# dhansmair/flamingo-mini

Hardware: AMD Instinct MI355X
Metric: images/sec (fwd+bwd) flamingo-mini bs=32 (higher is better)
Workload: dtype bf16

## Files before the change

flamingo-mini_amd/csrc/ff_rowwise.hip:

```cpp
#include "ff_common.h"
#include "ff_internal.h"

namespace ff {

#ifdef FF_XA_TIMELINE
__device__ unsigned long long g_ln_timeline[4096 * 8];
#define FF_LTL(i) do { if (threadIdx.x == 0 && blockIdx.x < 4096) g_ln_timeline[blockIdx.x * 8 + (i)] = __builtin_amdgcn_s_memrealtime(); } while (0)
#else
#define FF_LTL(i) do { } while (0)
#endif

template <typename T, int VEC> FF_DEV void ld(const T* p, float (&o)[VEC]) {
    if constexpr (VEC == 1) o[0] = to_f32(p[0]);
    else Vec<T>::load(p, o);
}
template <typename T, int VEC> FF_DEV void st(T* p, const float (&o)[VEC]) {
    if constexpr (VEC == 1) p[0] = from_f32<T>(o[0]);
    else Vec<T>::store(p, o);
}

template <typename T, int VEC>
__global__ __launch_bounds__(256) void ln_fwd_kernel(const LnArgs a_in, const T* __restrict__ x, const T* __restrict__ add,
                                                     const T* __restrict__ gamma, const T* __restrict__ beta, T* __restrict__ y,
                                                     float* __restrict__ mean, float* __restrict__ rstd) {
    const LnArgs a = fetch_args(a_in);
    pin_args(x, add, gamma, beta, y, mean, rstd);
    const int lane = threadIdx.x & 63;
    const int row = blockIdx.x * 4 + (threadIdx.x >> 6);
    if (row >= a.rows) return;
    const T* xr = x + a.x_map.off(row);
    const T* ar = nullptr;
    if (add) ar = add + (long long)((row % a.add_rows_per_seg) / a.add_div) * a.cols;
    const int nchunk = a.cols / VEC;
    float mu, rs;
    if (nchunk <= 4 * 64 && VEC > 1) {
        float v[4][VEC];
#pragma unroll
        for (int u = 0; u < 4; u++) {
            const int c = lane + 64 * u;
            if (c < nchunk) {
                ld<T, VEC>(xr + c * VEC, v[u]);
                if (ar) {
                    float t[VEC];
                    ld<T, VEC>(ar + c * VEC, t);
#pragma unroll
                    for (int i = 0; i < VEC; i++) v[u][i] += t[i];
                }
            }
        }
        if (a.stats_given) {
            mu = mean[row];
            rs = rstd[row];
        } else {
            float s = 0.f;
#pragma unroll
            for (int u = 0; u < 4; u++)
                if (lane + 64 * u < nchunk)
#pragma unroll
                    for (int i = 0; i < VEC; i++) s += v[u][i];
            mu = wave_sum(s) / (float)a.cols;
            float q = 0.f;
#pragma unroll
            for (int u = 0; u < 4; u++)
                if (lane + 64 * u < nchunk)
#pragma unroll
                    for (int i = 0; i < VEC; i++) q += (v[u][i] - mu) * (v[u][i] - mu);
            rs = rsqrtf(wave_sum(q) / (float)a.cols + a.eps);
            if (lane == 0 && mean) {
                mean[row] = mu;
                rstd[row] = rs;
            }
        }
        if (!y) return;
        T* yr = y + a.y_map.off(row);
#pragma unroll
        for (int u = 0; u < 4; u++) {
            const int c = lane + 64 * u;
            if (c < nchunk) {
                float g[VEC], b[VEC], o[VEC];
                ld<T, VEC>(gamma + c * VEC, g);
                ld<T, VEC>(beta + c * VEC, b);
#pragma unroll
                for (int i = 0; i < VEC; i++) o[i] = (v[u][i] - mu) * rs * g[i] + b[i];
                st<T, VEC>(yr + c * VEC, o);
            }
        }
        return;
    }
    if (a.stats_given) {
        mu = mean[row];
        rs = rstd[row];
    } else {
        float s = 0.f;
        for (int c = lane; c < nchunk; c += 64) {
            float v[VEC];
            ld<T, VEC>(xr + c * VEC, v);
            if (ar) {
                float t[VEC];
                ld<T, VEC>(ar + c * VEC, t);
#pragma unroll
                for (int i = 0; i < VEC; i++) v[i] += t[i];
            }
#pragma unroll
            for (int i = 0; i < VEC; i++) s += v[i];
        }
        mu = wave_sum(s) / (float)a.cols;
        float q = 0.f;
        for (int c = lane; c < nchunk; c += 64) {
            float v[VEC];
            ld<T, VEC>(xr + c * VEC, v);
            if (ar) {
                float t[VEC];
                ld<T, VEC>(ar + c * VEC, t);
#pragma unroll
                for (int i = 0; i < VEC; i++) v[i] += t[i];
            }
#pragma unroll
            for (int i = 0; i < VEC; i++) q += (v[i] - mu) * (v[i] - mu);
        }
        rs = rsqrtf(wave_sum(q) / (float)a.cols + a.eps);
        if (lane == 0 && mean) {
            mean[row] = mu;
            rstd[row] = rs;
        }
    }
    if (!y) return;
    T* yr = y + a.y_map.off(row);
    for (int c = lane; c < nchunk; c += 64) {
        float v[VEC], g[VEC], b[VEC];
        ld<T, VEC>(xr + c * VEC, v);
        if (ar) {
            float t[VEC];
            ld<T, VEC>(ar + c * VEC, t);
#pragma unroll
            for (int i = 0; i < VEC; i++) v[i] += t[i];
        }
        ld<T, VEC>(gamma + c * VEC, g);
        ld<T, VEC>(beta + c * VEC, b);
#pragma unroll
        for (int i = 0; i < VEC; i++) v[i] = (v[i] - mu) * rs * g[i] + b[i];
        st<T, VEC>(yr + c * VEC, v);
    }
}

template <typename T, int VEC>
__global__ __launch_bounds__(256) void ln_bwd_dx_kernel(const LnArgs a_in, const T* __restrict__ dy, const T* __restrict__ x,
                                                        const T* __restrict__ add, const T* __restrict__ gamma,
                                                        const float* __restrict__ mean, const float* __restrict__ rstd, T* dx,
                                                        const T* dx_res) {
    const LnArgs a = fetch_args(a_in);
    pin_args(dy, x, add, gamma, mean, rstd, dx, dx_res);
    const int lane = threadIdx.x & 63;
    const int row = blockIdx.x * 4 + (threadIdx.x >> 6);
    if (row >= a.rows) return;
    const T* xr = x + a.x_map.off(row);
    const T* dyr = dy + a.y_map.off(row);
    const T* ar = nullptr;
    if (add) ar = add + (long long)((row % a.add_rows_per_seg) / a.add_div) * a.cols;
    const float mu = mean[row], rs = rstd[row];
    const int nchunk = a.cols / VEC;
    float s1 = 0.f, s2 = 0.f;
    for (int c = lane; c < nchunk; c += 64) {
        float v[VEC], d[VEC], g[VEC];
        ld<T, VEC>(xr + c * VEC, v);
        if (ar) {
            float t[VEC];
            ld<T, VEC>(ar + c * VEC, t);
#pragma unroll
            for (int i = 0; i < VEC; i++) v[i] += t[i];
        }
        ld<T, VEC>(dyr + c * VEC, d);
        ld<T, VEC>(gamma + c * VEC, g);
#pragma unroll
        for (int i = 0; i < VEC; i++) {
            const float dyh = d[i] * g[i];
            s1 += dyh;
            s2 += dyh * (v[i] - mu) * rs;
        }
    }
    const float m1 = wave_sum(s1) / (float)a.cols, m2 = wave_sum(s2) / (float)a.cols;
    const long long doff = a.dx_map.off(row);
    for (int c = lane; c < nchunk; c += 64) {
        float v[VEC], d[VEC], g[VEC], o[VEC];
        ld<T, VEC>(xr + c * VEC, v);
        if (ar) {
            float t[VEC];
            ld<T, VEC>(ar + c * VEC, t);
#pragma unroll
            for (int i = 0; i < VEC; i++) v[i] += t[i];
        }
        ld<T, VEC>(dyr + c * VEC, d);
        ld<T, VEC>(gamma + c * VEC, g);
#pragma unroll
        for (int i = 0; i < VEC; i++) o[i] = rs * (d[i] * g[i] - m1 - (v[i] - mu) * rs * m2);
        if (dx_res) {
            float q[VEC];
            ld<T, VEC>(dx_res + doff + c * VEC, q);
#pragma unroll
            for (int i = 0; i < VEC; i++) o[i] += q[i];
        }
        st<T, VEC>(dx + doff + c * VEC, o);
    }
}


template <typename T, int VEC, int NCH>
__global__ __launch_bounds__(256) void ln_bwd_fused_kernel(const LnArgs a_in, const T* __restrict__ dy, const T* __restrict__ x,
                                                           const T* __restrict__ add, const T* __restrict__ gamma,
                                                           const float* __restrict__ mean, const float* __restrict__ rstd, T* dx,
                                                           const T* dx_res, const T* __restrict__ dot_a, const T* __restrict__ dot_b,
                                                           float* __restrict__ partial, int rows_per_block) {
    FF_LTL(0);
    const LnArgs a = fetch_args(a_in);
    pin_args(dy, x, add, gamma, mean, rstd, dx, dx_res, dot_a, dot_b, partial, rows_per_block);
    extern __shared__ __attribute__((aligned(16))) float sacc[];
    FF_LTL(1);
    __shared__ float red[4];
    const int lane = threadIdx.x & 63, w = threadIdx.x >> 6;
    const int nchunk = a.cols / VEC;
    float accg[NCH][VEC], accb[NCH][VEC];
#pragma unroll
    for (int i = 0; i < NCH; i++)
#pragma unroll
        for (int e = 0; e < VEC; e++) accg[i][e] = accb[i][e] = 0.f;
    float da = 0.f, db = 0.f;
    const int row_end = min(a.rows, (int)(blockIdx.x + 1) * rows_per_block);
    auto load_dy = [&](int row, const T* dyr, int c, float (&d)[VEC]) {
        if (a.dy_splits > 0) {
            const float* pp = (const float*)dy + (long long)row * a.cols + c * VEC;
#pragma unroll
            for (int e = 0; e < VEC; e++) d[e] = 0.f;
            for (int sp = 0; sp < a.dy_splits; sp++) {
#pragma unroll
                for (int e = 0; e < VEC; e += 4) {
                    const f32x4 q = *(const f32x4*)(pp + (long long)sp * a.dy_slab + e);
                    d[e] += q[0]; d[e + 1] += q[1]; d[e + 2] += q[2]; d[e + 3] += q[3];
                }
            }
        } else ld<T, VEC>(dyr + c * VEC, d);
    };
    for (int row = blockIdx.x * rows_per_block + w; row < row_end; row += 4) {
        const T* xr = x + a.x_map.off(row);
        const T* dyr = a.dy_splits > 0 ? dy : dy + a.y_map.off(row);
        const T* ar = add ? add + (long long)((row % a.add_rows_per_seg) / a.add_div) * a.cols : nullptr;
        const float mu = mean[row], rs = rstd[row];
        float s1 = 0.f, s2 = 0.f;
        constexpr bool KEEP = NCH <= 4;
        constexpr bool HOIST = KEEP && VEC > 1;
        float xk[KEEP ? NCH : 1][VEC], dk[KEEP ? NCH : 1][VEC];
        uint4 rq[HOIST ? NCH : 1], ra[HOIST ? NCH : 1], rb[HOIST ? NCH : 1];
        const long long doff = a.dx_map.off(row);
#pragma unroll
        for (int i = 0; i < NCH; i++) {
            const int c = lane + 64 * i;
            if (c < nchunk) {
                float v[VEC], d[VEC], g[VEC];
                ld<T, VEC>(xr + c * VEC, v);
                if (ar) {
                    float t[VEC];
                    ld<T, VEC>(ar + c * VEC, t);
#pragma unroll
                    for (int e = 0; e < VEC; e++) v[e] += t[e];
                }
                load_dy(row, dyr, c, d);
                ld<T, VEC>(gamma + c * VEC, g);
                if constexpr (HOIST) {
                    if (dx_res) rq[i] = *(const uint4*)(dx_res + doff + c * VEC);
                    if (dot_a) ra[i] = *(const uint4*)(dot_a + doff + c * VEC);
                    if (dot_b) rb[i] = *(const uint4*)(dot_b + doff + c * VEC);
                }
#pragma unroll
                for (int e = 0; e < VEC; e++) {
                    const float dyh = d[e] * g[e], xh = (v[e] - mu) * rs;
                    s1 += dyh;
                    s2 += dyh * xh;
                    if (KEEP) { xk[i][e] = xh; dk[i][e] = d[e]; }
                }
            }
        }
        const float m1 = wave_sum(s1) / (float)a.cols, m2 = wave_sum(s2) / (float)a.cols;
        auto unpack = [](const uint4& r, float (&o)[VEC]) {
            if constexpr (VEC > 1) {
                typedef typename Vec<T>::raw raw_t;
                const raw_t x = __builtin_bit_cast(raw_t, r);
#pragma unroll
                for (int e = 0; e < VEC; e++) o[e] = to_f32(x[e]);
            }
        };
#pragma unroll
        for (int i = 0; i < NCH; i++) {
            const int c = lane + 64 * i;
            if (c < nchunk) {
                float xh[VEC], d[VEC], g[VEC], o[VEC];
                if (KEEP) {
#pragma unroll
                    for (int e = 0; e < VEC; e++) { xh[e] = xk[i][e]; d[e] = dk[i][e]; }
                } else {
                    float v[VEC];
                    ld<T, VEC>(xr + c * VEC, v);
                    if (ar) {
                        float t[VEC];
                        ld<T, VEC>(ar + c * VEC, t);
#pragma unroll
                        for (int e = 0; e < VEC; e++) v[e] += t[e];
                    }
                    load_dy(row, dyr, c, d);
#pragma unroll
                    for (int e = 0; e < VEC; e++) xh[e] = (v[e] - mu) * rs;
                }
                ld<T, VEC>(gamma + c * VEC, g);
#pragma unroll
                for (int e = 0; e < VEC; e++) {
                    o[e] = rs * (d[e] * g[e] - m1 - xh[e] * m2);
                    accg[i][e] += d[e] * xh[e];
                    accb[i][e] += d[e];
                }
                if (dx_res) {
                    float q[VEC];
                    if constexpr (HOIST) unpack(rq[i], q);
                    else ld<T, VEC>(dx_res + doff + c * VEC, q);
                    if (dot_a) {
                        float u[VEC];
                        if constexpr (HOIST) unpack(ra[i], u);
                        else ld<T, VEC>(dot_a + doff + c * VEC, u);
#pragma unroll
                        for (int e = 0; e < VEC; e++) da += q[e] * u[e];
                    }
#pragma unroll
                    for (int e = 0; e < VEC; e++) o[e] += q[e];
                }
                if (dx) {
                    float r[VEC];
#pragma unroll
                    for (int e = 0; e < VEC; e++) r[e] = to_f32(from_f32<T>(o[e]));
                    if (dot_b) {
                        float u[VEC];
                        if constexpr (HOIST) unpack(rb[i], u);
                        else ld<T, VEC>(dot_b + doff + c * VEC, u);
#pragma unroll
                        for (int e = 0; e < VEC; e++) db += r[e] * u[e];
                    }
                    st<T, VEC>(dx + doff + c * VEC, o);
                }
            }
        }
    }
    FF_LTL(2);
    {
        float* mine = sacc + (size_t)w * 2 * a.cols;
#pragma unroll
        for (int i = 0; i < NCH; i++) {
            const int c = lane + 64 * i;
            if (c < nchunk) {
#pragma unroll
                for (int e = 0; e < VEC; e += 4) {
                    *(f32x4*)(mine + c * VEC + e) = f32x4{accg[i][e], accg[i][e + 1], accg[i][e + 2], accg[i][e + 3]};
                    *(f32x4*)(mine + a.cols + c * VEC + e) = f32x4{accb[i][e], accb[i][e + 1], accb[i][e + 2], accb[i][e + 3]};
                }
            }
        }
    }
    __syncthreads();
    FF_LTL(3);
    const long long P = 2LL * a.cols + 2;
    float* out = partial + (long long)blockIdx.x * P;
    for (int i = threadIdx.x * 4; i < 2 * a.cols; i += 256 * 4) {
        const f32x4 s0 = *(const f32x4*)(sacc + i), s1 = *(const f32x4*)(sacc + 2 * a.cols + i);
        const f32x4 s2 = *(const f32x4*)(sacc + 4 * a.cols + i), s3 = *(const f32x4*)(sacc + 6 * a.cols + i);
        float* o = out + i;
        o[0] = (s0[0] + s1[0]) + (s2[0] + s3[0]); o[1] = (s0[1] + s1[1]) + (s2[1] + s3[1]);
        o[2] = (s0[2] + s1[2]) + (s2[2] + s3[2]); o[3] = (s0[3] + s1[3]) + (s2[3] + s3[3]);
    }
    da = block_sum<4>(da, red);
    db = block_sum<4>(db, red);
    if (threadIdx.x == 0) { out[2 * a.cols] = da; out[2 * a.cols + 1] = db; }
    FF_LTL(4);
}

template <typename T>
FF_DEV void ln_final_body(int nblk, int cols, const float* __restrict__ partial, T* dgamma, T* dbeta, const T* alpha_a, T* out_a, const T* alpha_b,
                          T* out_b) {
    __shared__ float red[16][17];
    const int P = 2 * cols + 2;
    const int tx = threadIdx.x & 15, ty = threadIdx.x >> 4;
    const int idx = blockIdx.x * 16 + tx;
    float v[8] = {0.f, 0.f, 0.f, 0.f, 0.f, 0.f, 0.f, 0.f};
    if (idx < P) {
        int b = ty;
        for (; b + 7 * 16 < nblk; b += 8 * 16) {
#pragma unroll
            for (int u = 0; u < 8; u++) v[u] += partial[(long long)(b + 16 * u) * P + idx];
        }
        for (; b < nblk; b += 16) v[0] += partial[(long long)b * P + idx];
    }
    red[ty][tx] = ((v[0] + v[1]) + (v[2] + v[3])) + ((v[4] + v[5]) + (v[6] + v[7]));
    __syncthreads();
    if (ty == 0 && idx < P) {
        float s = 0.f;
#pragma unroll
        for (int u = 0; u < 16; u++) s += red[u][tx];
        const float v = s;
        if (idx < cols) { if (dgamma) dgamma[idx] = from_f32<T>(v); }
        else if (idx < 2 * cols) { if (dbeta) dbeta[idx - cols] = from_f32<T>(v); }
        else if (idx == 2 * cols) {
            if (out_a) { const float t = tanhf(to_f32(alpha_a[0])); out_a[0] = from_f32<T>(v * (1.f - t * t)); }
        } else if (out_b) { const float t = tanhf(to_f32(alpha_b[0])); out_b[0] = from_f32<T>(v * (1.f - t * t)); }
    }
}
template <typename T>
// ... 9 lines not shown
__global__ __launch_bounds__(256) void ln_bwd_final_multi_kernel(const LnFinishTable t) {
    const LnPending& e = t.s[blockIdx.y];
    if ((int)blockIdx.x * 16 >= 2 * e.cols + 2) return;
    ln_final_body<T>(e.nblk, e.cols, e.partial, (T*)e.dgamma, (T*)e.dbeta, (const T*)e.alpha_a, (T*)e.out_a, (const T*)e.alpha_b, (T*)e.out_b);
}

struct ColReduceArgs {
    int rows, cols;
    RowMap x_map, y_map;
    int rows_per_batch, rows_per_group, n_batch;
    int add_rows_per_seg, add_div;
    int rows_per_split, nsplit, ngroups;
};

template <typename T, int VEC, int MODE>
__global__ __launch_bounds__(256) void col_reduce_kernel(const ColReduceArgs a_in, const T* __restrict__ x, const T* __restrict__ dy,
                                                         const T* __restrict__ add, const float* __restrict__ mean,
                                                         const float* __restrict__ rstd, float* __restrict__ partial) {
    const ColReduceArgs a = fetch_args(a_in);
    pin_args(x, dy, add, mean, rstd, partial);
    constexpr int NS = MODE == 1 ? 2 : 1;
    __shared__ float red[4][NS][64 * VEC];
    const int tx = threadIdx.x & 63, ty = threadIdx.x >> 6;
    const int col = (blockIdx.x * 64 + tx) * VEC;
    const int g = blockIdx.y, split = blockIdx.z;
    float acc[NS][VEC];
#pragma unroll
    for (int s = 0; s < NS; s++)
#pragma unroll
        for (int i = 0; i < VEC; i++) acc[s][i] = 0.f;
    if (col < a.cols) {
        const int n_g = a.n_batch * a.rows_per_group;
        const int i_end = min(n_g, (split + 1) * a.rows_per_split);
        for (int i = split * a.rows_per_split + ty; i < i_end; i += 4) {
            const int bi = i / a.rows_per_group, j = i - bi * a.rows_per_group;
            const int row = bi * a.rows_per_batch + g * a.rows_per_group + j;
            if (row >= a.rows) continue;
            float v[VEC];
            ld<T, VEC>(x + a.x_map.off(row) + col, v);
            if (MODE == 0) {
#pragma unroll
                for (int e = 0; e < VEC; e++) acc[0][e] += v[e];
            } else {
                if (add) {
                    float t[VEC];
                    ld<T, VEC>(add + (long long)((row % a.add_rows_per_seg) / a.add_div) * a.cols + col, t);
#pragma unroll
                    for (int e = 0; e < VEC; e++) v[e] += t[e];
                }
                float d[VEC];
                ld<T, VEC>(dy + a.y_map.off(row) + col, d);
                const float mu = mean[row], rs = rstd[row];
#pragma unroll
                for (int e = 0; e < VEC; e++) {
                    acc[0][e] += d[e] * (v[e] - mu) * rs;
                    acc[1][e] += d[e];
                }
            }
        }
    }
#pragma unroll
    for (int s = 0; s < NS; s++)
#pragma unroll
        for (int e = 0; e < VEC; e++) red[ty][s][tx * VEC + e] = acc[s][e];
    __syncthreads();
    if (ty == 0 && col < a.cols) {
#pragma unroll
        for (int s = 0; s < NS; s++)
#pragma unroll
            for (int e = 0; e < VEC; e++) {
                const float v = red[0][s][tx * VEC + e] + red[1][s][tx * VEC + e] + red[2][s][tx * VEC + e] + red[3][s][tx * VEC + e];
                partial[(((long long)split * a.ngroups + g) * NS + s) * a.cols + col + e] = v;
            }
    }
}

template <typename T>
__global__ __launch_bounds__(256) void col_reduce_final_kernel(int nsplit, int ngroups, int nslots, int cols,
                                                               const float* __restrict__ partial, T* out0, T* out1) {
    pin_args(nsplit, ngroups, nslots, cols, partial, out0, out1);
    const long long total = (long long)ngroups * nslots * cols;
    for (long long idx = (long long)blockIdx.x * 256 + threadIdx.x; idx < total; idx += (long long)gridDim.x * 256) {
        float v0 = 0.f, v1 = 0.f, v2 = 0.f, v3 = 0.f;
        int s = 0;
        for (; s + 4 <= nsplit; s += 4) {
            v0 += partial[(long long)s * total + idx];
            v1 += partial[(long long)(s + 1) * total + idx];
            v2 += partial[(long long)(s + 2) * total + idx];
            v3 += partial[(long long)(s + 3) * total + idx];
        }
        for (; s < nsplit; s++) v0 += partial[(long long)s * total + idx];
        const float v = (v0 + v1) + (v2 + v3);
        const int c = (int)(idx % cols);
        const long long gs = idx / cols;
        const int slot = (int)(gs % nslots), g = (int)(gs / nslots);
        T* out = slot == 0 ? out0 : out1;
        out[(long long)g * cols + c] = from_f32<T>(v);
    }
}

template <typename T, int VEC>
__global__ __launch_bounds__(256) void dot_partial_kernel(long long n, const T* __restrict__ a, const T* __restrict__ b,
                                                          float* __restrict__ partial) {
    pin_args(n, a, b, partial);
    __shared__ float red[4];
// ... 36 lines not shown
              size_t ws_bytes, hipStream_t st_);

static bool vec_ok(int dtype, int cols, std::initializer_list<RowMap> maps, std::initializer_list<const void*> ptrs) {
    const int n = dtype == FF_DTYPE_BF16 ? 8 : 4;
    if (cols % n) return false;
    for (const RowMap& m : maps)
        if (m.ld % n || (m.rows_per_seg > 0 && m.seg_stride % n)) return false;
    for (const void* p : ptrs)
        if (p && (uintptr_t)p % 16) return false;
    return true;
}

#define FF_DISPATCH_T_VEC(dtype, vec, ...)                 \
    do {                                                    \
        if ((dtype) == FF_DTYPE_BF16) {                     \
            typedef bf16 T;                                 \
            if (vec) { constexpr int VEC = 8; __VA_ARGS__; }       \
            else { constexpr int VEC = 1; __VA_ARGS__; }           \
        } else {                                            \
            typedef float T;                                \
            if (vec) { constexpr int VEC = 4; __VA_ARGS__; }       \
            else { constexpr int VEC = 1; __VA_ARGS__; }           \
        }                                                   \
    } while (0)

int layernorm_fwd(const LnArgs& a, const void* x, const void* add, const void* gamma, const void* beta, void* y, float* mean,
                  float* rstd, hipStream_t st_) {
    FF_CHECK(a.rows > 0 && a.cols > 0 && x, FF_ERR_SHAPE, "layernorm_fwd: bad shape rows=%d cols=%d", a.rows, a.cols);
    FF_CHECK(!a.stats_given || (mean && rstd), FF_ERR_SHAPE, "layernorm_fwd: stats_given without statistics");
    FF_CHECK(!y || (gamma && beta), FF_ERR_SHAPE, "layernorm_fwd: gamma/beta missing");
    FF_CHECK(!add || (a.add_rows_per_seg > 0 && a.add_div > 0), FF_ERR_SHAPE, "layernorm_fwd: addend needs add_rows_per_seg/add_div");
    const bool v = vec_ok(a.dtype, a.cols, {a.x_map, a.y_map}, {x, add, gamma, beta, y});
    const int grid = cdiv(a.rows, 4);
    FF_DISPATCH_T_VEC(a.dtype, v, ln_fwd_kernel<T, VEC><<<dim3(grid), dim3(256), 0, st_>>>(a, (const T*)x, (const T*)add, (const T*)gamma, (const T*)beta, (T*)y, mean, rstd));
    return check_launch("ln_fwd");
}

static void split_plan(int n_rows_in_group, int col_blocks, int ngroups, int& rows_per_split, int& nsplit) {
    int target = std::max(1, 512 / std::max(1, col_blocks * ngroups));
    nsplit = std::max(1, std::min(std::min(target, 32), cdiv(n_rows_in_group, 32)));
    rows_per_split = cdiv(n_rows_in_group, nsplit);
    nsplit = cdiv(n_rows_in_group, rows_per_split);
}

static size_t col_reduce_ws(int n_rows_in_group, int cols, int ngroups, int nslots) {
    int rps, ns;
    split_plan(n_rows_in_group, 1, ngroups, rps, ns);
    return (size_t)ns * ngroups * nslots * cols * sizeof(float);
}


static int ln_fused_blocks(int rows, int& rows_per_block) {
    rows_per_block = std::max(4, (cdiv(rows, 256) + 3) / 4 * 4);
    return cdiv(rows, rows_per_block);
}
static bool ln_fused_ok(int dtype, int cols, bool vec) {
    if (!vec) return false;
    const int n = dtype == FF_DTYPE_BF16 ? 8 : 4;
    return cdiv(cols / n, 64) <= 8 && (size_t)8 * cols * sizeof(float) <= 150 * 1024;
}
size_t layernorm_bwd_workspace(int rows, int cols) {
    int rpb;
    const size_t fused = (size_t)ln_fused_blocks(rows, rpb) * (2 * (size_t)cols + 2) * sizeof(float);
    return std::max(fused, col_reduce_ws(rows, cols, 1, 2));
}

bool layernorm_bwd_deferrable(int dtype, int cols) { return cols % (dtype == FF_DTYPE_BF16 ? 8 : 4) == 0 && ln_fused_ok(dtype, cols, true); }
int layernorm_bwd_partial_blocks(int rows) {
    int rpb;
    return ln_fused_blocks(rows, rpb);
}
size_t layernorm_bwd_partial_bytes(int rows, int cols) { return (size_t)layernorm_bwd_partial_blocks(rows) * (2 * (size_t)cols + 2) * sizeof(float); }

template <typename T, int VEC>
static int launch_ln_fused(const LnArgs& a, const void* dy, const void* x, const void* add, const void* gamma, const float* mean,
                           const float* rstd, void* dx, const void* dx_res, const LnDots& dots, void* dgamma, void* dbeta, float* partial,
                           hipStream_t st_, LnPending* pending) {
    int rpb;
    const int nblk = ln_fused_blocks(a.rows, rpb);
    const int nch = cdiv(a.cols / VEC, 64);
    const size_t lds = (size_t)8 * a.cols * sizeof(float);
#define FF_LN_LAUNCH(NCH)                                                                                                                 \
    do {                                                                                                                                  \
        if (lds > 48 * 1024) {                                                                                                            \
            static bool attr[64] = {};                                                                                                    \
            int dev = 0;                                                                                                                  \
            (void)hipGetDevice(&dev);                                                                                                     \
            if (dev < 0 || dev >= 64 || !attr[dev]) {                                                                                     \
                hipFuncSetAttribute((const void*)ln_bwd_fused_kernel<T, VEC, NCH>, hipFuncAttributeMaxDynamicSharedMemorySize, 150 * 1024); \
                if (dev >= 0 && dev < 64) attr[dev] = true;                                                                               \
            }                                                                                                                             \
        }                                                                                                                                 \
        ln_bwd_fused_kernel<T, VEC, NCH><<<dim3(nblk), dim3(256), lds, st_>>>(a, (const T*)dy, (const T*)x, (const T*)add, (const T*)gamma, \
                                                                              mean, rstd, (T*)dx, (const T*)dx_res, (const T*)dots.a,     \
                                                                              (const T*)dots.b, partial, rpb);                            \
    } while (0)
    if (nch <= 2) FF_LN_LAUNCH(2);
    else if (nch <= 4) FF_LN_LAUNCH(4);
    else FF_LN_LAUNCH(8);
#undef FF_LN_LAUNCH
    FF_TRY(check_launch("ln_bwd_fused"));
    if (pending) {
        pending->partial = partial; pending->nblk = nblk; pending->cols = a.cols; pending->dgamma = dgamma; pending->dbeta = dbeta;
        pending->alpha_a = dots.alpha_a; pending->out_a = dots.out_a; pending->alpha_b = dots.alpha_b; pending->out_b = dots.out_b;
        return FF_OK;
    }
    const int P = 2 * a.cols + 2;
    ln_bwd_final_kernel<T><<<dim3(cdiv(P, 16)), dim3(256), 0, st_>>>(nblk, a.cols, partial, (T*)dgamma, (T*)dbeta, (const T*)dots.alpha_a,
                                                                     (T*)dots.out_a, (const T*)dots.alpha_b, (T*)dots.out_b);
    return check_launch("ln_bwd_final");
}

int layernorm_bwd(const LnArgs& a, const void* dy, const void* x, const void* add, const void* gamma, const float* mean,
                  const float* rstd, void* dx, const void* dx_residual, void* dgamma, void* dbeta, void* ws, size_t ws_bytes,
                  hipStream_t st_, const LnDots* dots_in, LnPending* pending) {
    FF_CHECK(a.rows > 0 && a.cols > 0 && dy && x && gamma && mean && rstd, FF_ERR_SHAPE, "layernorm_bwd: null/shape");
    if (pending) *pending = LnPending{};
    FF_CHECK(!add || (a.add_rows_per_seg > 0 && a.add_div > 0), FF_ERR_SHAPE, "layernorm_bwd: addend needs add_rows_per_seg/add_div");
    const LnDots dots = dots_in ? *dots_in : LnDots{};
    FF_CHECK(!dots.a || dx_residual, FF_ERR_SHAPE, "layernorm_bwd: dot_a is taken against dx_residual");
    FF_CHECK(!dots.b || dx, FF_ERR_SHAPE, "layernorm_bwd: dot_b is taken against dx");
    const bool v = vec_ok(a.dtype, a.cols, {a.x_map, a.y_map, a.dx_map}, {x, add, gamma, dy, dx, dx_residual, dots.a, dots.b});
    FF_CHECK(a.dy_splits == 0 || (ln_fused_ok(a.dtype, a.cols, v) && (dgamma || dots.a || dots.b) && a.cols % 4 == 0), FF_ERR_UNSUPPORTED,
             "layernorm_bwd: summing split-K slabs needs the one-pass kernel");
    if (ln_fused_ok(a.dtype, a.cols, v) && (dgamma || dots.a || dots.b)) {
        FF_CHECK(!dgamma == !dbeta, FF_ERR_SHAPE, "layernorm_bwd: dgamma and dbeta come together");
        int rpb;
        const size_t need = (size_t)ln_fused_blocks(a.rows, rpb) * (2 * (size_t)a.cols + 2) * sizeof(float);
        FF_CHECK(ws && ws_bytes >= need, FF_ERR_WORKSPACE, "layernorm_bwd workspace: need %zu have %zu", need, ws_bytes);
        if (a.dtype == FF_DTYPE_BF16) return launch_ln_fused<bf16, 8>(a, dy, x, add, gamma, mean, rstd, dx, dx_residual, dots, dgamma, dbeta, (float*)ws, st_, pending);
        return launch_ln_fused<float, 4>(a, dy, x, add, gamma, mean, rstd, dx, dx_residual, dots, dgamma, dbeta, (float*)ws, st_, pending);
    }
// ... 165 lines not shown
```

Measured before the change: 802.0.

## Specialize layernorm kernels and prefetch row operands ahead of compute

Layernorm forward is templated on chunk count and the presence of an addend, and issues all row, gamma and beta loads up front before the reductions. The fused backward kernel is specialized on chunk count, dy split count and the optional operand set, and uses a request/consume structure so the next row's global loads can be issued before the current row is computed. It also reads split fp32 dy slabs directly and reduces them in registers. Global loads and stores go through address-space-1 casts, and a general kernel is kept as a fallback. The cost is more template instantiations, higher register pressure, and dispatch logic that must match the caller's split and option combinations.

```diff
diff --git a/flamingo-mini_amd/csrc/ff_rowwise.hip b/flamingo-mini_amd/csrc/ff_rowwise.hip
--- a/flamingo-mini_amd/csrc/ff_rowwise.hip
+++ b/flamingo-mini_amd/csrc/ff_rowwise.hip
@@ -1,3 +1,4 @@
+#include <type_traits>
 #include "ff_common.h"
 #include "ff_internal.h"
 
@@ -10,16 +11,34 @@
 #define FF_LTL(i) do { } while (0)
 #endif
 
+template <typename V, typename P> FF_DEV V gld(const P* p) { return *(const __attribute__((address_space(1))) V*)p; }
+template <typename V, typename P> FF_DEV void gst(P* p, const V& v) { *(__attribute__((address_space(1))) V*)p = v; }
+template <typename R, int N> FF_DEV void unpack(const R& r, float (&o)[N]) {
+#pragma unroll
+    for (int e = 0; e < N; e++) o[e] = to_f32(r[e]);
+}
+
+template <typename T, int VEC> using Piece = typename std::conditional<VEC == 1, T, typename Vec<T>::raw>::type;
+template <int VEC, typename R> FF_DEV void as_floats(const R& r, float (&o)[VEC]) {
+    if constexpr (VEC == 1) o[0] = to_f32(r);
+    else unpack(r, o);
+}
+
 template <typename T, int VEC> FF_DEV void ld(const T* p, float (&o)[VEC]) {
-    if constexpr (VEC == 1) o[0] = to_f32(p[0]);
-    else Vec<T>::load(p, o);
+    if constexpr (VEC == 1) o[0] = to_f32(gld<T>(p));
+    else unpack(gld<typename Vec<T>::raw>(p), o);
 }
 template <typename T, int VEC> FF_DEV void st(T* p, const float (&o)[VEC]) {
-    if constexpr (VEC == 1) p[0] = from_f32<T>(o[0]);
-    else Vec<T>::store(p, o);
-}
-
-template <typename T, int VEC>
+    if constexpr (VEC == 1) gst<T>(p, from_f32<T>(o[0]));
+    else {
+        typename Vec<T>::raw v;
+#pragma unroll
+        for (int i = 0; i < VEC; i++) v[i] = from_f32<T>(o[i]);
+        gst(p, v);
+    }
+}
+
+template <typename T, int VEC, int NCH, bool ADD>
 __global__ __launch_bounds__(256) void ln_fwd_kernel(const LnArgs a_in, const T* __restrict__ x, const T* __restrict__ add,
                                                      const T* __restrict__ gamma, const T* __restrict__ beta, T* __restrict__ y,
                                                      float* __restrict__ mean, float* __restrict__ rstd) {
@@ -30,72 +49,87 @@
     if (row >= a.rows) return;
     const T* xr = x + a.x_map.off(row);
     const T* ar = nullptr;
-    if (add) ar = add + (long long)((row % a.add_rows_per_seg) / a.add_div) * a.cols;
+    if (ADD) ar = add + (long long)((row % a.add_rows_per_seg) / a.add_div) * a.cols;
     const int nchunk = a.cols / VEC;
     float mu, rs;
-    if (nchunk <= 4 * 64 && VEC > 1) {
-        float v[4][VEC];
-#pragma unroll
-        for (int u = 0; u < 4; u++) {
-            const int c = lane + 64 * u;
-            if (c < nchunk) {
-                ld<T, VEC>(xr + c * VEC, v[u]);
-                if (ar) {
+    if constexpr (NCH > 0) {
+        typedef typename Vec<T>::raw raw_t;
+        raw_t xv[NCH], av[ADD ? NCH : 1], gv[NCH], bv[NCH];
+        int off[NCH];
+        if (a.stats_given) {
+            mu = gld<float>(mean + row);
+            rs = gld<float>(rstd + row);
+        }
+#pragma unroll
+        for (int u = 0; u < NCH; u++) {
+            off[u] = (lane + 64 * u < nchunk ? lane + 64 * u : 0) * VEC;
+            xv[u] = gld<raw_t>(xr + off[u]);
+            if constexpr (ADD) av[u] = gld<raw_t>(ar + off[u]);
+        }
+        if (y) {
+#pragma unroll
+            for (int u = 0; u < NCH; u++) {
+                gv[u] = gld<raw_t>(gamma + off[u]);
+                bv[u] = gld<raw_t>(beta + off[u]);
+            }
+        }
+        float v[NCH][VEC];
+#pragma unroll
+        for (int u = 0; u < NCH; u++) {
+            if (lane + 64 * u < nchunk) {
+                unpack(xv[u], v[u]);
+                if constexpr (ADD) {
                     float t[VEC];
-                    ld<T, VEC>(ar + c * VEC, t);
+                    unpack(av[u], t);
 #pragma unroll
                     for (int i = 0; i < VEC; i++) v[u][i] += t[i];
                 }
             }
         }
-        if (a.stats_given) {
-            mu = mean[row];
-            rs = rstd[row];
-        } else {
+        if (!a.stats_given) {
             float s = 0.f;
 #pragma unroll
-            for (int u = 0; u < 4; u++)
+            for (int u = 0; u < NCH; u++)
                 if (lane + 64 * u < nchunk)
 #pragma unroll
                     for (int i = 0; i < VEC; i++) s += v[u][i];
             mu = wave_sum(s) / (float)a.cols;
             float q = 0.f;
 #pragma unroll
-            for (int u = 0; u < 4; u++)
+            for (int u = 0; u < NCH; u++)
                 if (lane + 64 * u < nchunk)
 #pragma unroll
                     for (int i = 0; i < VEC; i++) q += (v[u][i] - mu) * (v[u][i] - mu);
             rs = rsqrtf(wave_sum(q) / (float)a.cols + a.eps);
             if (lane == 0 && mean) {
-                mean[row] = mu;
-                rstd[row] = rs;
+                gst(mean + row, mu);
+                gst(rstd + row, rs);
             }
         }
         if (!y) return;
         T* yr = y + a.y_map.off(row);
 #pragma unroll
-        for (int u = 0; u < 4; u++) {
-            const int c = lane + 64 * u;
-            if (c < nchunk) {
+        for (int u = 0; u < NCH; u++) {
+            if (lane + 64 * u < nchunk) {
                 float g[VEC], b[VEC], o[VEC];
-                ld<T, VEC>(gamma + c * VEC, g);
-                ld<T, VEC>(beta + c * VEC, b);
+                unpack(gv[u], g);
+                unpack(bv[u], b);
 #pragma unroll
                 for (int i = 0; i < VEC; i++) o[i] = (v[u][i] - mu) * rs * g[i] + b[i];
-                st<T, VEC>(yr + c * VEC, o);
+                st<T, VEC>(yr + off[u], o);
             }
         }
         return;
     }
     if (a.stats_given) {
-        mu = mean[row];
-        rs = rstd[row];
+        mu = gld<float>(mean + row);
+        rs = gld<float>(rstd + row);
     } else {
         float s = 0.f;
         for (int c = lane; c < nchunk; c += 64) {
             float v[VEC];
             ld<T, VEC>(xr + c * VEC, v);
-            if (ar) {
+            if (ADD) {
                 float t[VEC];
                 ld<T, VEC>(ar + c * VEC, t);
 #pragma unroll
@@ -109,7 +143,7 @@
         for (int c = lane; c < nchunk; c += 64) {
             float v[VEC];
             ld<T, VEC>(xr + c * VEC, v);
-            if (ar) {
+            if (ADD) {
                 float t[VEC];
                 ld<T, VEC>(ar + c * VEC, t);
 #pragma unroll
@@ -120,8 +154,8 @@
         }
         rs = rsqrtf(wave_sum(q) / (float)a.cols + a.eps);
         if (lane == 0 && mean) {
-            mean[row] = mu;
-            rstd[row] = rs;
+            gst(mean + row, mu);
+            gst(rstd + row, rs);
         }
     }
     if (!y) return;
@@ -129,7 +163,7 @@
     for (int c = lane; c < nchunk; c += 64) {
         float v[VEC], g[VEC], b[VEC];
         ld<T, VEC>(xr + c * VEC, v);
-        if (ar) {
+        if (ADD) {
             float t[VEC];
             ld<T, VEC>(ar + c * VEC, t);
 #pragma unroll
@@ -157,20 +191,24 @@
     const T* dyr = dy + a.y_map.off(row);
     const T* ar = nullptr;
     if (add) ar = add + (long long)((row % a.add_rows_per_seg) / a.add_div) * a.cols;
-    const float mu = mean[row], rs = rstd[row];
+    const float mu = gld<float>(mean + row), rs = gld<float>(rstd + row);
     const int nchunk = a.cols / VEC;
+    typedef Piece<T, VEC> raw_t;
     float s1 = 0.f, s2 = 0.f;
     for (int c = lane; c < nchunk; c += 64) {
+        const raw_t xv = gld<raw_t>(xr + c * VEC), dv = gld<raw_t>(dyr + c * VEC), gv = gld<raw_t>(gamma + c * VEC);
+        raw_t tv;
+        if (add) tv = gld<raw_t>(ar + c * VEC);
         float v[VEC], d[VEC], g[VEC];
-        ld<T, VEC>(xr + c * VEC, v);
-        if (ar) {
+        as_floats(xv, v);
+        if (add) {
             float t[VEC];
-            ld<T, VEC>(ar + c * VEC, t);
+            as_floats(tv, t);
 #pragma unroll
             for (int i = 0; i < VEC; i++) v[i] += t[i];
         }
-        ld<T, VEC>(dyr + c * VEC, d);
-        ld<T, VEC>(gamma + c * VEC, g);
+        as_floats(dv, d);
+        as_floats(gv, g);
 #pragma unroll
         for (int i = 0; i < VEC; i++) {
             const float dyh = d[i] * g[i];
@@ -181,21 +219,25 @@
     const float m1 = wave_sum(s1) / (float)a.cols, m2 = wave_sum(s2) / (float)a.cols;
     const long long doff = a.dx_map.off(row);
     for (int c = lane; c < nchunk; c += 64) {
+        const raw_t xv = gld<raw_t>(xr + c * VEC), dv = gld<raw_t>(dyr + c * VEC), gv = gld<raw_t>(gamma + c * VEC);
+        raw_t tv, qv;
+        if (add) tv = gld<raw_t>(ar + c * VEC);
+        if (dx_res) qv = gld<raw_t>(dx_res + doff + c * VEC);
         float v[VEC], d[VEC], g[VEC], o[VEC];
-        ld<T, VEC>(xr + c * VEC, v);
-        if (ar) {
+        as_floats(xv, v);
+        if (add) {
             float t[VEC];
-            ld<T, VEC>(ar + c * VEC, t);
+            as_floats(tv, t);
 #pragma unroll
             for (int i = 0; i < VEC; i++) v[i] += t[i];
         }
-        ld<T, VEC>(dyr + c * VEC, d);
-        ld<T, VEC>(gamma + c * VEC, g);
+        as_floats(dv, d);
+        as_floats(gv, g);
 #pragma unroll
         for (int i = 0; i < VEC; i++) o[i] = rs * (d[i] * g[i] - m1 - (v[i] - mu) * rs * m2);
         if (dx_res) {
             float q[VEC];
-            ld<T, VEC>(dx_res + doff + c * VEC, q);
+            as_floats(qv, q);
 #pragma unroll
             for (int i = 0; i < VEC; i++) o[i] += q[i];
         }
@@ -204,12 +246,53 @@
 }
 
 
-template <typename T, int VEC, int NCH>
+template <int VEC, int NCH>
+FF_DEV void ln_bwd_block_out(int cols, const float (&accg)[NCH][VEC], const float (&accb)[NCH][VEC], float da, float db, float* partial,
+                             float* sacc, float* red) {
+    FF_LTL(2);
+    const int lane = threadIdx.x & 63, w = threadIdx.x >> 6;
+    const int nchunk = cols / VEC;
+    {
+        float* mine = sacc + (size_t)w * 2 * cols;
+#pragma unroll
+        for (int i = 0; i < NCH; i++) {
+            const int c = lane + 64 * i;
+            if (c < nchunk) {
+#pragma unroll
+                for (int e = 0; e < VEC; e += 4) {
+                    *(f32x4*)(mine + c * VEC + e) = f32x4{accg[i][e], accg[i][e + 1], accg[i][e + 2], accg[i][e + 3]};
+                    *(f32x4*)(mine + cols + c * VEC + e) = f32x4{accb[i][e], accb[i][e + 1], accb[i][e + 2], accb[i][e + 3]};
+                }
+            }
+        }
+    }
+    __syncthreads();
+    FF_LTL(3);
+    const long long P = 2LL * cols + 2;
+    float* out = partial + (long long)blockIdx.x * P;
+    for (int i = threadIdx.x * 4; i < 2 * cols; i += 256 * 4) {
+        const f32x4 s0 = *(const f32x4*)(sacc + i), s1 = *(const f32x4*)(sacc + 2 * cols + i);
+        const f32x4 s2 = *(const f32x4*)(sacc + 4 * cols + i), s3 = *(const f32x4*)(sacc + 6 * cols + i);
+        float* o = out + i;
+        gst(o, f32x2{(s0[0] + s1[0]) + (s2[0] + s3[0]), (s0[1] + s1[1]) + (s2[1] + s3[1])});
+        gst(o + 2, f32x2{(s0[2] + s1[2]) + (s2[2] + s3[2]), (s0[3] + s1[3]) + (s2[3] + s3[3])});
+    }
+    da = block_sum<4>(da, red);
+    db = block_sum<4>(db, red);
+    if (threadIdx.x == 0) { gst(out + 2 * cols, da); gst(out + 2 * cols + 1, db); }
+    FF_LTL(4);
+}
+
+template <typename T, int NCH, int SPL, int OPT>
 __global__ __launch_bounds__(256) void ln_bwd_fused_kernel(const LnArgs a_in, const T* __restrict__ dy, const T* __restrict__ x,
                                                            const T* __restrict__ add, const T* __restrict__ gamma,
                                                            const float* __restrict__ mean, const float* __restrict__ rstd, T* dx,
                                                            const T* dx_res, const T* __restrict__ dot_a, const T* __restrict__ dot_b,
                                                            float* __restrict__ partial, int rows_per_block) {
+    constexpr int VEC = Vec<T>::N;
+    constexpr bool ADD = (OPT & 1) != 0, RES = (OPT & 2) != 0, DA = (OPT & 4) != 0, DB = (OPT & 8) != 0;
+    static_assert(NCH <= 4 && (!DA || RES), "dot_a is taken against dx_res");
+    typedef typename Vec<T>::raw raw_t;
     FF_LTL(0);
     const LnArgs a = fetch_args(a_in);
     pin_args(dy, x, add, gamma, mean, rstd, dx, dx_res, dot_a, dot_b, partial, rows_per_block);
@@ -225,17 +308,190 @@
         for (int e = 0; e < VEC; e++) accg[i][e] = accb[i][e] = 0.f;
     float da = 0.f, db = 0.f;
     const int row_end = min(a.rows, (int)(blockIdx.x + 1) * rows_per_block);
+    int off[NCH];
+#pragma unroll
+    for (int i = 0; i < NCH; i++) off[i] = (lane + 64 * i < nchunk ? lane + 64 * i : 0) * VEC;
+    struct Row {
+        raw_t g[NCH], x[NCH], ad[ADD ? NCH : 1], dy[SPL ? 1 : NCH], q[RES ? NCH : 1], ua[DA ? NCH : 1], ub[DB ? NCH : 1];
+        f32x4 slab[SPL ? NCH : 1][SPL ? SPL : 1][VEC / 4];
+        float mu, rs;
+        long long doff;
+    };
+    auto request = [&](int row, Row& r) {
+        const T* xr = x + a.x_map.off(row);
+        r.doff = a.dx_map.off(row);
+        r.mu = gld<float>(mean + row);
+        r.rs = gld<float>(rstd + row);
+#pragma unroll
+        for (int i = 0; i < NCH; i++) {
+            r.g[i] = gld<raw_t>(gamma + off[i]);
+            r.x[i] = gld<raw_t>(xr + off[i]);
+        }
+        if constexpr (ADD) {
+            const T* ar = add + (long long)((row % a.add_rows_per_seg) / a.add_div) * a.cols;
+#pragma unroll
+            for (int i = 0; i < NCH; i++) r.ad[i] = gld<raw_t>(ar + off[i]);
+        }
+        if constexpr (SPL > 0) {
+            const float* pp = (const float*)dy + (long long)row * a.cols;
+#pragma unroll
+            for (int i = 0; i < NCH; i++)
+#pragma unroll
+                for (int sp = 0; sp < SPL; sp++)
+#pragma unroll
+                    for (int e = 0; e < VEC; e += 4) r.slab[i][sp][e / 4] = gld<f32x4>(pp + (long long)sp * a.dy_slab + off[i] + e);
+        } else {
+            const T* dyr = dy + a.y_map.off(row);
+#pragma unroll
+            for (int i = 0; i < NCH; i++) r.dy[i] = gld<raw_t>(dyr + off[i]);
+        }
+#pragma unroll
+        for (int i = 0; i < NCH; i++) {
+            if constexpr (RES) r.q[i] = gld<raw_t>(dx_res + r.doff + off[i]);
+            if constexpr (DA) r.ua[i] = gld<raw_t>(dot_a + r.doff + off[i]);
+            if constexpr (DB) r.ub[i] = gld<raw_t>(dot_b + r.doff + off[i]);
+        }
+    };
+    auto consume = [&](const Row& r) {
+        const float mu = r.mu, rs = r.rs;
+        float s1 = 0.f, s2 = 0.f;
+        float xk[NCH][VEC], dk[NCH][VEC];
+#pragma unroll
+        for (int i = 0; i < NCH; i++) {
+            if (lane + 64 * i < nchunk) {
+                float v[VEC], d[VEC], g[VEC];
+                unpack(r.x[i], v);
+                if constexpr (ADD) {
+                    float t[VEC];
+                    unpack(r.ad[i], t);
+#pragma unroll
+                    for (int e = 0; e < VEC; e++) v[e] += t[e];
+                }
+                if constexpr (SPL > 0) {
+#pragma unroll
+                    for (int e = 0; e < VEC; e++) d[e] = 0.f;
+#pragma unroll
+                    for (int sp = 0; sp < SPL; sp++)
+#pragma unroll
+                        for (int e = 0; e < VEC; e += 4) {
+                            const f32x4 q = r.slab[i][sp][e / 4];
+                            d[e] += q[0]; d[e + 1] += q[1]; d[e + 2] += q[2]; d[e + 3] += q[3];
+                        }
+                } else unpack(r.dy[i], d);
+                unpack(r.g[i], g);
+#pragma unroll
+                for (int e = 0; e < VEC; e++) {
+                    const float dyh = d[e] * g[e], xh = (v[e] - mu) * rs;
+                    s1 += dyh;
+                    s2 += dyh * xh;
+                    xk[i][e] = xh; dk[i][e] = d[e];
+                }
+            }
+        }
+        const float m1 = wave_sum(s1) / (float)a.cols, m2 = wave_sum(s2) / (float)a.cols;
+#pragma unroll
+        for (int i = 0; i < NCH; i++) {
+            if (lane + 64 * i < nchunk) {
+                float xh[VEC], d[VEC], g[VEC], o[VEC];
+#pragma unroll
+                for (int e = 0; e < VEC; e++) { xh[e] = xk[i][e]; d[e] = dk[i][e]; }
+                unpack(r.g[i], g);
+#pragma unroll
+                for (int e = 0; e < VEC; e++) {
+                    o[e] = rs * (d[e] * g[e] - m1 - xh[e] * m2);
+                    accg[i][e] += d[e] * xh[e];
+                    accb[i][e] += d[e];
+                }
+                if constexpr (RES) {
+                    float q[VEC];
+                    unpack(r.q[i], q);
+                    if constexpr (DA) {
+                        float u[VEC];
+                        unpack(r.ua[i], u);
+#pragma unroll
+                        for (int e = 0; e < VEC; e++) da += q[e] * u[e];
+                    }
+                    {
+#pragma clang fp contract(off)
+#pragma unroll
+                        for (int e = 0; e < VEC; e++) o[e] = o[e] + q[e];
+                    }
+                }
+                if (dx) {
+                    if constexpr (DB) {
+                        float u[VEC];
+                        unpack(r.ub[i], u);
+#pragma unroll
+                        for (int e = 0; e < VEC; e++) db += to_f32(from_f32<T>(o[e])) * u[e];
+                    }
+                    st<T, VEC>(dx + r.doff + off[i], o);
+                }
+            }
+        }
+    };
+    int row = blockIdx.x * rows_per_block + w;
+    if (row < row_end) {
+        Row cur;
+        request(row, cur);
+        for (;;) {
+            const bool more = row + 4 < row_end;
+            if constexpr (SPL == 0) {
+                Row nxt;
+                if (more) request(row + 4, nxt);
+                consume(cur);
+                if (!more) break;
+                cur = nxt;
+            } else {
+                consume(cur);
+                if (!more) break;
+                request(row + 4, cur);
+            }
+            row += 4;
+        }
+    }
+    ln_bwd_block_out<VEC, NCH>(a.cols, accg, accb, da, db, partial, sacc, red);
+}
+
+template <typename T, int VEC, int NCH>
+__global__ __launch_bounds__(256) void ln_bwd_fused_general_kernel(const LnArgs a_in, const T* __restrict__ dy, const T* __restrict__ x,
+                                                                   const T* __restrict__ add, const T* __restrict__ gamma,
+                                                                   const float* __restrict__ mean, const float* __restrict__ rstd, T* dx,
+                                                                   const T* dx_res, const T* __restrict__ dot_a, const T* __restrict__ dot_b,
+                                                                   float* __restrict__ partial, int rows_per_block) {
+    FF_LTL(0);
+    const LnArgs a = fetch_args(a_in);
+    pin_args(dy, x, add, gamma, mean, rstd, dx, dx_res, dot_a, dot_b, partial, rows_per_block);
+    extern __shared__ __attribute__((aligned(16))) float sacc[];
+    FF_LTL(1);
+    __shared__ float red[4];
+    const int lane = threadIdx.x & 63, w = threadIdx.x >> 6;
+    const int nchunk = a.cols / VEC;
+    float accg[NCH][VEC], accb[NCH][VEC];
+#pragma unroll
+    for (int i = 0; i < NCH; i++)
+#pragma unroll
+        for (int e = 0; e < VEC; e++) accg[i][e] = accb[i][e] = 0.f;
+    float da = 0.f, db = 0.f;
+    const int row_end = min(a.rows, (int)(blockIdx.x + 1) * rows_per_block);
     auto load_dy = [&](int row, const T* dyr, int c, float (&d)[VEC]) {
         if (a.dy_splits > 0) {
             const float* pp = (const float*)dy + (long long)row * a.cols + c * VEC;
 #pragma unroll
             for (int e = 0; e < VEC; e++) d[e] = 0.f;
-            for (int sp = 0; sp < a.dy_splits; sp++) {
-#pragma unroll
-                for (int e = 0; e < VEC; e += 4) {
-                    const f32x4 q = *(const f32x4*)(pp + (long long)sp * a.dy_slab + e);
-                    d[e] += q[0]; d[e + 1] += q[1]; d[e + 2] += q[2]; d[e + 3] += q[3];
-                }
+            for (int sp = 0; sp < a.dy_splits; sp += 4) {
+                f32x4 q[4][VEC / 4];
+#pragma unroll
+                for (int u = 0; u < 4; u++)
+                    if (sp + u < a.dy_splits)
+#pragma unroll
+                        for (int e = 0; e < VEC; e += 4) q[u][e / 4] = gld<f32x4>(pp + (long long)(sp + u) * a.dy_slab + e);
+#pragma unroll
+                for (int u = 0; u < 4; u++)
+                    if (sp + u < a.dy_splits)
+#pragma unroll
+                        for (int e = 0; e < VEC; e += 4) {
+                            d[e] += q[u][e / 4][0]; d[e + 1] += q[u][e / 4][1]; d[e + 2] += q[u][e / 4][2]; d[e + 3] += q[u][e / 4][3];
+                        }
             }
         } else ld<T, VEC>(dyr + c * VEC, d);
     };
@@ -243,12 +499,13 @@
         const T* xr = x + a.x_map.off(row);
         const T* dyr = a.dy_splits > 0 ? dy : dy + a.y_map.off(row);
         const T* ar = add ? add + (long long)((row % a.add_rows_per_seg) / a.add_div) * a.cols : nullptr;
-        const float mu = mean[row], rs = rstd[row];
+        const float mu = gld<float>(mean + row), rs = gld<float>(rstd + row);
         float s1 = 0.f, s2 = 0.f;
         constexpr bool KEEP = NCH <= 4;
         constexpr bool HOIST = KEEP && VEC > 1;
         float xk[KEEP ? NCH : 1][VEC], dk[KEEP ? NCH : 1][VEC];
-        uint4 rq[HOIST ? NCH : 1], ra[HOIST ? NCH : 1], rb[HOIST ? NCH : 1];
+        typedef typename Vec<T>::raw raw_t;
+        raw_t rq[HOIST ? NCH : 1], ra[HOIST ? NCH : 1], rb[HOIST ? NCH : 1];
         const long long doff = a.dx_map.off(row);
 #pragma unroll
         for (int i = 0; i < NCH; i++) {
@@ -265,9 +522,9 @@
                 load_dy(row, dyr, c, d);
                 ld<T, VEC>(gamma + c * VEC, g);
                 if constexpr (HOIST) {
-                    if (dx_res) rq[i] = *(const uint4*)(dx_res + doff + c * VEC);
-                    if (dot_a) ra[i] = *(const uint4*)(dot_a + doff + c * VEC);
-                    if (dot_b) rb[i] = *(const uint4*)(dot_b + doff + c * VEC);
+                    if (dx_res) rq[i] = gld<raw_t>(dx_res + doff + c * VEC);
+                    if (dot_a) ra[i] = gld<raw_t>(dot_a + doff + c * VEC);
+                    if (dot_b) rb[i] = gld<raw_t>(dot_b + doff + c * VEC);
                 }
 #pragma unroll
                 for (int e = 0; e < VEC; e++) {
@@ -279,14 +536,6 @@
             }
         }
         const float m1 = wave_sum(s1) / (float)a.cols, m2 = wave_sum(s2) / (float)a.cols;
-        auto unpack = [](const uint4& r, float (&o)[VEC]) {
-            if constexpr (VEC > 1) {
-                typedef typename Vec<T>::raw raw_t;
-                const raw_t x = __builtin_bit_cast(raw_t, r);
-#pragma unroll
-                for (int e = 0; e < VEC; e++) o[e] = to_f32(x[e]);
-            }
-        };
 #pragma unroll
         for (int i = 0; i < NCH; i++) {
             const int c = lane + 64 * i;
@@ -345,36 +594,7 @@
             }
         }
     }
-    FF_LTL(2);
-    {
-        float* mine = sacc + (size_t)w * 2 * a.cols;
-#pragma unroll
-        for (int i = 0; i < NCH; i++) {
-            const int c = lane + 64 * i;
-            if (c < nchunk) {
-#pragma unroll
-                for (int e = 0; e < VEC; e += 4) {
-                    *(f32x4*)(mine + c * VEC + e) = f32x4{accg[i][e], accg[i][e + 1], accg[i][e + 2], accg[i][e + 3]};
-                    *(f32x4*)(mine + a.cols + c * VEC + e) = f32x4{accb[i][e], accb[i][e + 1], accb[i][e + 2], accb[i][e + 3]};
-                }
-            }
-        }
-    }
-    __syncthreads();
-    FF_LTL(3);
-    const long long P = 2LL * a.cols + 2;
-    float* out = partial + (long long)blockIdx.x * P;
-    for (int i = threadIdx.x * 4; i < 2 * a.cols; i += 256 * 4) {
-        const f32x4 s0 = *(const f32x4*)(sacc + i), s1 = *(const f32x4*)(sacc + 2 * a.cols + i);
-        const f32x4 s2 = *(const f32x4*)(sacc + 4 * a.cols + i), s3 = *(const f32x4*)(sacc + 6 * a.cols + i);
-        float* o = out + i;
-        o[0] = (s0[0] + s1[0]) + (s2[0] + s3[0]); o[1] = (s0[1] + s1[1]) + (s2[1] + s3[1]);
-        o[2] = (s0[2] + s1[2]) + (s2[2] + s3[2]); o[3] = (s0[3] + s1[3]) + (s2[3] + s3[3]);
-    }
-    da = block_sum<4>(da, red);
-    db = block_sum<4>(db, red);
-    if (threadIdx.x == 0) { out[2 * a.cols] = da; out[2 * a.cols + 1] = db; }
-    FF_LTL(4);
+    ln_bwd_block_out<VEC, NCH>(a.cols, accg, accb, da, db, partial, sacc, red);
 }
 
 template <typename T>
@@ -450,29 +670,55 @@
     if (col < a.cols) {
         const int n_g = a.n_batch * a.rows_per_group;
         const int i_end = min(n_g, (split + 1) * a.rows_per_split);
-        for (int i = split * a.rows_per_split + ty; i < i_end; i += 4) {
-            const int bi = i / a.rows_per_group, j = i - bi * a.rows_per_group;
-            const int row = bi * a.rows_per_batch + g * a.rows_per_group + j;
-            if (row >= a.rows) continue;
-            float v[VEC];
-            ld<T, VEC>(x + a.x_map.off(row) + col, v);
-            if (MODE == 0) {
-#pragma unroll
-                for (int e = 0; e < VEC; e++) acc[0][e] += v[e];
-            } else {
+        constexpr int U = MODE == 0 ? 8 : 4;
+        typedef Piece<T, VEC> raw_t;
+        for (int i0 = split * a.rows_per_split + ty; i0 < i_end; i0 += 4 * U) {
+            raw_t xv[U], tv[MODE == 1 ? U : 1], dv[MODE == 1 ? U : 1];
+            float mu[MODE == 1 ? U : 1], rs[MODE == 1 ? U : 1];
+            int rowv[U];
+            bool ok[U];
+#pragma unroll
+            for (int u = 0; u < U; u++) {
+                const int i = i0 + 4 * u;
+                const int bi = i / a.rows_per_group, j = i - bi * a.rows_per_group;
+                const int row = bi * a.rows_per_batch + g * a.rows_per_group + j;
+                ok[u] = i < i_end && row < a.rows;
+                rowv[u] = ok[u] ? row : 0;
+                xv[u] = gld<raw_t>(x + a.x_map.off(rowv[u]) + col);
+                if constexpr (MODE == 1) {
+                    dv[u] = gld<raw_t>(dy + a.y_map.off(rowv[u]) + col);
+                    mu[u] = gld<float>(mean + rowv[u]);
+                    rs[u] = gld<float>(rstd + rowv[u]);
+                }
+            }
+            if constexpr (MODE == 1) {
                 if (add) {
-                    float t[VEC];
-                    ld<T, VEC>(add + (long long)((row % a.add_rows_per_seg) / a.add_div) * a.cols + col, t);
-#pragma unroll
-                    for (int e = 0; e < VEC; e++) v[e] += t[e];
-                }
-                float d[VEC];
-                ld<T, VEC>(dy + a.y_map.off(row) + col, d);
-                const float mu = mean[row], rs = rstd[row];
-#pragma unroll
-                for (int e = 0; e < VEC; e++) {
-                    acc[0][e] += d[e] * (v[e] - mu) * rs;
-                    acc[1][e] += d[e];
+#pragma unroll
+                    for (int u = 0; u < U; u++) tv[u] = gld<raw_t>(add + (long long)((rowv[u] % a.add_rows_per_seg) / a.add_div) * a.cols + col);
+                }
+            }
+#pragma unroll
+            for (int u = 0; u < U; u++) {
+                if (!ok[u]) continue;
+                float v[VEC];
+                as_floats(xv[u], v);
+                if constexpr (MODE == 0) {
+#pragma unroll
+                    for (int e = 0; e < VEC; e++) acc[0][e] += v[e];
+                } else {
+                    if (add) {
+                        float t[VEC];
+                        as_floats(tv[u], t);
+#pragma unroll
+                        for (int e = 0; e < VEC; e++) v[e] += t[e];
+                    }
+                    float d[VEC];
+                    as_floats(dv[u], d);
+#pragma unroll
+                    for (int e = 0; e < VEC; e++) {
+                        acc[0][e] += d[e] * (v[e] - mu[u]) * rs[u];
+                        acc[1][e] += d[e];
+                    }
                 }
             }
         }
@@ -488,7 +734,7 @@
 #pragma unroll
             for (int e = 0; e < VEC; e++) {
                 const float v = red[0][s][tx * VEC + e] + red[1][s][tx * VEC + e] + red[2][s][tx * VEC + e] + red[3][s][tx * VEC + e];
-                partial[(((long long)split * a.ngroups + g) * NS + s) * a.cols + col + e] = v;
+                gst(partial + (((long long)split * a.ngroups + g) * NS + s) * a.cols + col + e, v);
             }
     }
 }
@@ -591,7 +837,18 @@
     FF_CHECK(!add || (a.add_rows_per_seg > 0 && a.add_div > 0), FF_ERR_SHAPE, "layernorm_fwd: addend needs add_rows_per_seg/add_div");
     const bool v = vec_ok(a.dtype, a.cols, {a.x_map, a.y_map}, {x, add, gamma, beta, y});
     const int grid = cdiv(a.rows, 4);
-    FF_DISPATCH_T_VEC(a.dtype, v, ln_fwd_kernel<T, VEC><<<dim3(grid), dim3(256), 0, st_>>>(a, (const T*)x, (const T*)add, (const T*)gamma, (const T*)beta, (T*)y, mean, rstd));
+    const int nch = v ? cdiv(a.cols / (a.dtype == FF_DTYPE_BF16 ? 8 : 4), 64) : 0;
+#define FF_LN_FWD(NCH, ADD) ln_fwd_kernel<T, VEC, NCH, ADD><<<dim3(grid), dim3(256), 0, st_>>>(a, (const T*)x, (const T*)add, (const T*)gamma, (const T*)beta, (T*)y, mean, rstd)
+#define FF_LN_FWD_NCH(NCH) do { if (add) FF_LN_FWD(NCH, true); else FF_LN_FWD(NCH, false); } while (0)
+    FF_DISPATCH_T_VEC(a.dtype, v,
+                      if constexpr (VEC == 1) FF_LN_FWD_NCH(0);
+                      else if (nch > 4) FF_LN_FWD_NCH(0);
+                      else if (nch == 1) FF_LN_FWD_NCH(1);
+                      else if (nch == 2) FF_LN_FWD_NCH(2);
+                      else if (nch == 3) FF_LN_FWD_NCH(3);
+                      else FF_LN_FWD_NCH(4));
+#undef FF_LN_FWD_NCH
+#undef FF_LN_FWD
     return check_launch("ln_fwd");
 }
 
@@ -630,6 +887,17 @@
     return ln_fused_blocks(rows, rpb);
 }
 size_t layernorm_bwd_partial_bytes(int rows, int cols) { return (size_t)layernorm_bwd_partial_blocks(rows) * (2 * (size_t)cols + 2) * sizeof(float); }
+
+template <auto KERNEL> static void ln_fused_lds_limit(size_t lds) {
+    if (lds <= 48 * 1024) return;
+    static bool attr[64] = {};
+    int dev = 0;
+    (void)hipGetDevice(&dev);
+    if (dev < 0 || dev >= 64 || !attr[dev]) {
+        (void)hipFuncSetAttribute((const void*)KERNEL, hipFuncAttributeMaxDynamicSharedMemorySize, 150 * 1024);
+        if (dev >= 0 && dev < 64) attr[dev] = true;
+    }
+}
 
 template <typename T, int VEC>
 static int launch_ln_fused(const LnArgs& a, const void* dy, const void* x, const void* add, const void* gamma, const float* mean,
@@ -639,24 +907,31 @@
     const int nblk = ln_fused_blocks(a.rows, rpb);
     const int nch = cdiv(a.cols / VEC, 64);
     const size_t lds = (size_t)8 * a.cols * sizeof(float);
-#define FF_LN_LAUNCH(NCH)                                                                                                                 \
+    const int opt = (add ? 1 : 0) | (dx_res ? 2 : 0) | (dots.a ? 4 : 0) | (dots.b ? 8 : 0);
+    const int spl = a.dy_splits;
+    bool launched = false;
+#define FF_LN_LAUNCH(...)                                                                                                                 \
     do {                                                                                                                                  \
-        if (lds > 48 * 1024) {                                                                                                            \
-            static bool attr[64] = {};                                                                                                    \
-            int dev = 0;                                                                                                                  \
-            (void)hipGetDevice(&dev);                                                                                                     \
-            if (dev < 0 || dev >= 64 || !attr[dev]) {                                                                                     \
-                hipFuncSetAttribute((const void*)ln_bwd_fused_kernel<T, VEC, NCH>, hipFuncAttributeMaxDynamicSharedMemorySize, 150 * 1024); \
-                if (dev >= 0 && dev < 64) attr[dev] = true;                                                                               \
-            }                                                                                                                             \
-        }                                                                                                                                 \
-        ln_bwd_fused_kernel<T, VEC, NCH><<<dim3(nblk), dim3(256), lds, st_>>>(a, (const T*)dy, (const T*)x, (const T*)add, (const T*)gamma, \
-                                                                              mean, rstd, (T*)dx, (const T*)dx_res, (const T*)dots.a,     \
-                                                                              (const T*)dots.b, partial, rpb);                            \
+        ln_fused_lds_limit<__VA_ARGS__>(lds);                                                                                             \
+        __VA_ARGS__<<<dim3(nblk), dim3(256), lds, st_>>>(a, (const T*)dy, (const T*)x, (const T*)add, (const T*)gamma, mean, rstd, (T*)dx, \
+                                                         (const T*)dx_res, (const T*)dots.a, (const T*)dots.b, partial, rpb);             \
+        launched = true;                                                                                                                  \
     } while (0)
-    if (nch <= 2) FF_LN_LAUNCH(2);
-    else if (nch <= 4) FF_LN_LAUNCH(4);
-    else FF_LN_LAUNCH(8);
+#define FF_LN_CASE(NCH, SPL, OPT) \
+    if (!launched && nch <= NCH && spl == SPL && opt == OPT) FF_LN_LAUNCH(ln_bwd_fused_kernel<T, NCH, SPL, OPT>)
+#define FF_LN_CASES(NCH)                                                                                                   \
+    FF_LN_CASE(NCH, 0, 0); FF_LN_CASE(NCH, 0, 1); FF_LN_CASE(NCH, 0, 2); FF_LN_CASE(NCH, 0, 3); FF_LN_CASE(NCH, 0, 14); \
+    FF_LN_CASE(NCH, 2, 14); FF_LN_CASE(NCH, 3, 14); FF_LN_CASE(NCH, 4, 14); FF_LN_CASE(NCH, 8, 14)
+    FF_LN_CASES(2);
+    FF_LN_CASES(3);
+    FF_LN_CASES(4);
+    if (!launched) {
+        if (nch <= 2) FF_LN_LAUNCH(ln_bwd_fused_general_kernel<T, VEC, 2>);
+        else if (nch <= 4) FF_LN_LAUNCH(ln_bwd_fused_general_kernel<T, VEC, 4>);
+        else FF_LN_LAUNCH(ln_bwd_fused_general_kernel<T, VEC, 8>);
+    }
+#undef FF_LN_CASES
+#undef FF_LN_CASE
 #undef FF_LN_LAUNCH
     FF_TRY(check_launch("ln_bwd_fused"));
     if (pending) {
```

Result: no change. 809.7 (median of 6 runs) (+1.0%).
